# jkulhanek/viewformer

Hardware: NVIDIA H100
Metric: novel views/sec (128x128, 9-ctx) (higher is better)
Workload: dtype f32 encoder (bit-exact codes) + bf16 transformer/decoder

## Files before the change

### viewformer_b200/csrc/vf_tc_gemm.cu

```cuda
#include "vf_wgmma.cuh"
#include <stdlib.h>

namespace {
using namespace vftc;

constexpr int BLOCK_M = 128;
constexpr int ROW_BYTES = 128;
constexpr int A_STAGE_BYTES = BLOCK_M * ROW_BYTES;
constexpr int NUM_EPI_WARPS = 8;
constexpr int NUM_MMA_THREADS = 32 * NUM_EPI_WARPS;
constexpr int NUM_THREADS = NUM_MMA_THREADS + 128;

struct TcParams {
    CUtensorMap tmA, tmB;
    int conv;
    int M, Ncols;
    int num_k_blocks;
    int batch2;
    int tiles_m, tiles_n, total_tiles;
    int a_bm1, a_bm2, b_bm1, b_bm2;
    int TW, TH, TN, tiles_x, tiles_y, OH, OW, Nimg, cin_blocks, bk_elems;
    int tap_dy[9], tap_dx[9], tap_coff[9];
    int gemm_koff;
    int causal_block, causal_skip_n;
    float alpha;
    const float* bias;
    int bias_mode, act;
    const float* residual;
    float* C_f32;
    __nv_bfloat16* C_bf16;
    long long ldc, c_sb1, c_sb2;
    int vec_ok;
    int halo;
    double* gn_sums;
    int gn_groups, gn_cpg, gn_rows_per_img;
    int exact;
    int exact_kc;
    int exact_clog;
    int exact_kpp;
    int exact_lo_b;
    const float2* norm_mr;
    const float* norm_gamma;
    const float* norm_beta;
    int norm_groups, norm_cpg, norm_swish;
};

constexpr float EXACT_LO_SCALE = 1.0f / 2048.0f;

struct TileInfo {
    int m0, n0, b1, b2, img0, oy0, ox0, nkb;
    bool skip;
};

__device__ __forceinline__ TileInfo decode_tile(const TcParams& p, int t, int block_n) {
    TileInfo ti;
    const int n_tile = t % p.tiles_n;
    const int r = t / p.tiles_n;
    const int m_tile = r % p.tiles_m;
    const int bz = r / p.tiles_m;
    ti.b1 = bz / p.batch2;
    ti.b2 = bz % p.batch2;
    ti.m0 = m_tile * BLOCK_M;
    ti.n0 = n_tile * block_n;
    ti.nkb = p.num_k_blocks;
    ti.skip = false;
    if (p.causal_block > 0) {
        const int lim = ((ti.m0 + BLOCK_M - 1) / p.causal_block + 1) * p.causal_block;
        if (p.causal_skip_n) {
            ti.skip = ti.n0 >= lim;
        } else {
            const int kb = (lim + p.bk_elems - 1) / p.bk_elems;
            if (kb < ti.nkb) ti.nkb = kb;
        }
    }
    ti.img0 = ti.oy0 = ti.ox0 = 0;
    if (p.conv) {
        const int tx = m_tile % p.tiles_x;
        const int q = m_tile / p.tiles_x;
        ti.img0 = (q / p.tiles_y) * p.TN;
        ti.oy0 = (q % p.tiles_y) * p.TH;
        ti.ox0 = tx * p.TW;
    }
    return ti;
}

constexpr int HALO_BYTES = 23552;
__host__ __device__ constexpr int halo_buffers(bool exact) { return exact ? 4 : 2; }
__host__ __device__ constexpr int halo_slots(bool exact) { return exact ? 4 : 6; }
__host__ __device__ constexpr int operand_bytes(int stages, int stage_bytes, int b_stage_bytes, bool exact) {
    return stages * stage_bytes > halo_buffers(exact) * HALO_BYTES + halo_slots(exact) * b_stage_bytes
               ? stages * stage_bytes
               : halo_buffers(exact) * HALO_BYTES + halo_slots(exact) * b_stage_bytes;
}
constexpr int MAX_STAGES = 8;
template <int kBlockN, int kStages, bool kExact>
__host__ __device__ constexpr int tc_smem_bytes() {
    return operand_bytes(kStages, A_STAGE_BYTES + kBlockN * ROW_BYTES, kBlockN * ROW_BYTES, kExact) +
           NUM_EPI_WARPS * 32 * (kBlockN / 2 + 4) * 4  + 1024  + 8 * (2 * MAX_STAGES + 8) ;
}

__device__ __forceinline__ void prefetch_residual_l2(const TcParams& p, const TileInfo& ti, int block_n) {
    const int tw = min(p.TW, p.OW - ti.ox0);
    const uint32_t bytes = (uint32_t)(((long long)(tw - 1) * p.ldc + block_n) * 4);
    for (int r = 0; r < p.TN * p.TH; ++r) {
        const int img = ti.img0 + r / p.TH, oy = ti.oy0 + r % p.TH;
        if (img >= p.Nimg || oy >= p.OH) continue;
        const float* src = p.residual + ((long long)(img * p.OH + oy) * p.OW + ti.ox0) * p.ldc + ti.n0;
        asm volatile("cp.async.bulk.prefetch.L2.global [%0], %1;" ::"l"(src), "r"(bytes) : "memory");
    }
}

__device__ __forceinline__ void normalise_halo(const TcParams& p, uint8_t* tile, int cb, int img, int oy0, int ox0, int tid) {
    const int rows = (p.TW + 2) * (p.TH + 2);
    for (int idx = tid; idx < rows * 8; idx += NUM_MMA_THREADS) {
        const int r = idx >> 3, pc = idx & 7;
        const int py = r / (p.TW + 2), px = r - py * (p.TW + 2);
        const int iy = oy0 - 1 + py, ix = ox0 - 1 + px;
        if (iy < 0 || iy >= p.OH || ix < 0 || ix >= p.OW) continue;
        const int c0 = cb * 64 + ((pc ^ (r & 7)) << 3);
        uint4* ptr = reinterpret_cast<uint4*>(tile + r * ROW_BYTES + pc * 16);
        const uint4 v = *ptr;
        uint32_t w[4] = {v.x, v.y, v.z, v.w};
#pragma unroll
        for (int k = 0; k < 4; ++k) {
            const int c = c0 + 2 * k;
            const float2 ma = __ldg(p.norm_mr + (img * p.norm_groups + c / p.norm_cpg));
            const float2 mb = __ldg(p.norm_mr + (img * p.norm_groups + (c + 1) / p.norm_cpg));
            const float sa = ma.y * __ldg(p.norm_gamma + c), sb = mb.y * __ldg(p.norm_gamma + c + 1);
            float a = __uint_as_float(w[k] << 16), b = __uint_as_float(w[k] & 0xffff0000u);
            a = fmaf(a, sa, __ldg(p.norm_beta + c) - ma.x * sa);
            b = fmaf(b, sb, __ldg(p.norm_beta + c + 1) - mb.x * sb);
            if (p.norm_swish == 1) {
                a = __fdividef(a, 1.0f + __expf(-a));
                b = __fdividef(b, 1.0f + __expf(-b));
            }
            __nv_bfloat162 o = __floats2bfloat162_rn(a, b);
            w[k] = *reinterpret_cast<uint32_t*>(&o);
            if (p.norm_swish == 2) {
                uint32_t h, th;
                asm("mul.rn.bf16x2 %0, %1, %2;" : "=r"(h) : "r"(w[k]), "r"(0x3f003f00u));
                asm("tanh.approx.bf16x2 %0, %1;" : "=r"(th) : "r"(h));
                asm("fma.rn.bf16x2 %0, %1, %2, %1;" : "=r"(w[k]) : "r"(h), "r"(th));
            }
        }
        *ptr = make_uint4(w[0], w[1], w[2], w[3]);
    }
}

template <int kBlockN, int kStages, WgKind kKind>
__global__ void __launch_bounds__(NUM_THREADS, 1) tc_gemm_kernel(const __grid_constant__ TcParams p) {
    constexpr int B_STAGE_BYTES = kBlockN * ROW_BYTES;
    constexpr int STAGE_BYTES = A_STAGE_BYTES + B_STAGE_BYTES;
    constexpr int K_STEPS = 4;
    constexpr int HALF_N = kBlockN / 2;
    constexpr int STG_LD = HALF_N + 4;
    constexpr int STG_BYTES = NUM_EPI_WARPS * 32 * STG_LD * 4;
    constexpr int NACC = kBlockN / 2;
    constexpr bool kExact = kKind == F16;

    extern __shared__ uint8_t smem_raw[];
    uint8_t* smem = reinterpret_cast<uint8_t*>((reinterpret_cast<uintptr_t>(smem_raw) + 1023) & ~(uintptr_t)1023);
    constexpr int OPER_BYTES = operand_bytes(kStages, STAGE_BYTES, B_STAGE_BYTES, kExact);
    float* staging = reinterpret_cast<float*>(smem + OPER_BYTES);
    uint64_t* full_bar = reinterpret_cast<uint64_t*>(smem + OPER_BYTES + STG_BYTES);
    uint64_t* empty_bar = full_bar + MAX_STAGES;
    constexpr int NHB = halo_buffers(kExact);
    uint64_t* a_full_bar = empty_bar + MAX_STAGES;
    uint64_t* a_empty_bar = a_full_bar + NHB;
    constexpr int NG = kStages;
    constexpr int NGH = halo_slots(kExact);
    uint8_t* halo_b_base = smem + NHB * HALO_BYTES;

    const int warp = threadIdx.x >> 5;
    const int lane = threadIdx.x & 31;

    if (threadIdx.x == 0) {
        prefetch_tmap(&p.tmA);
        prefetch_tmap(&p.tmB);
        for (int s = 0; s < MAX_STAGES; ++s) {
            mbar_init(&full_bar[s], 1);
            mbar_init(&empty_bar[s], NUM_MMA_THREADS);
        }
        for (int a = 0; a < NHB; ++a) {
            mbar_init(&a_full_bar[a], 1);
            mbar_init(&a_empty_bar[a], NUM_MMA_THREADS);
        }
        mbar_fence_init();
    }
    __syncthreads();

    if (warp >= NUM_EPI_WARPS) {
        setmaxnreg_dec<40>();
        if (warp == NUM_EPI_WARPS && elect_one()) {
            int stage = 0;
            uint32_t phase = 0;
            int ab = 0;
            uint32_t aphase = 0, tpar = 0;
            for (int t = blockIdx.x; t < p.total_tiles; t += gridDim.x, tpar ^= 1) {
                const TileInfo ti = decode_tile(p, t, kBlockN);
                if (ti.skip) continue;
                const uint32_t halo_bytes = (uint32_t)((p.TW + 2) * (p.TH + 2)) * ROW_BYTES;
                if (kExact && p.halo) {
                    auto load_halves = [&](int h) {
                        for (int cb = 0; cb < p.cin_blocks; ++cb) {
                            const int hb = 2 * h + cb;
                            mbar_wait(&a_empty_bar[hb], tpar ^ 1, "vf_tc_gemm producer(halo)");
                            mbar_expect_tx(&a_full_bar[hb], halo_bytes);
                            tma_load_4d(smem + hb * HALO_BYTES, &p.tmA, &a_full_bar[hb], (h ? 0 : p.exact_clog) + cb * p.bk_elems,
                                        ti.ox0 - 1, ti.oy0 - 1, ti.img0);
                        }
                    };
                    load_halves(0);
                    if (p.residual && p.vec_ok && ti.n0 + kBlockN <= p.Ncols) prefetch_residual_l2(p, ti, kBlockN);
                    int j = 0, tap = 0, cb = 0;
                    for (int kb = 0; kb < ti.nkb; ++kb) {
                        if (kb == NGH) load_halves(1);
                        mbar_wait(&empty_bar[stage], phase ^ 1, "vf_tc_gemm producer");
                        mbar_expect_tx(&full_bar[stage], (uint32_t)B_STAGE_BYTES);
                        tma_load_4d(halo_b_base + stage * B_STAGE_BYTES, &p.tmB, &full_bar[stage],
                                    ((tap * 2 + (j == 1 ? 1 : 0)) * p.cin_blocks + cb) * p.bk_elems, ti.n0, 0, 0);
                        if (++cb == p.cin_blocks) { cb = 0; if (++tap == 9) { tap = 0; ++j; } }
                        if (++stage == NGH) { stage = 0; phase ^= 1; }
                    }
                    continue;
                }
                if (p.halo) {
                    const int nkb = 9 * p.cin_blocks;
                    int tap = 0, cb = 0;
                    for (int kb = 0; kb < nkb; ++kb) {
                        mbar_wait(&empty_bar[stage], phase ^ 1, "vf_tc_gemm producer");
                        mbar_expect_tx(&full_bar[stage], (uint32_t)B_STAGE_BYTES);
                        if (tap == 0) {
                            mbar_wait(&a_empty_bar[ab], aphase ^ 1, "vf_tc_gemm producer(halo)");
                            mbar_expect_tx(&a_full_bar[ab], halo_bytes);
                            tma_load_4d(smem + ab * HALO_BYTES, &p.tmA, &a_full_bar[ab], cb * p.bk_elems, ti.ox0 - 1, ti.oy0 - 1, ti.img0);
                            if (++ab == 2) { ab = 0; aphase ^= 1; }
                        }
                        tma_load_4d(halo_b_base + stage * B_STAGE_BYTES, &p.tmB, &full_bar[stage], (tap * p.cin_blocks + cb) * p.bk_elems,
                                    ti.n0, 0, 0);
                        if (++tap == 9) { tap = 0; ++cb; }
                        if (++stage == NGH) { stage = 0; phase ^= 1; }
                    }
                    continue;
                }
                if (kExact && p.conv && p.residual && p.vec_ok && ti.n0 + kBlockN <= p.Ncols) prefetch_residual_l2(p, ti, kBlockN);
                for (int kb = 0; kb < ti.nkb; ++kb) {
                    mbar_wait(&empty_bar[stage], phase ^ 1, "vf_tc_gemm producer");
                    mbar_expect_tx(&full_bar[stage], (uint32_t)STAGE_BYTES);
                    uint8_t* sa = smem + stage * STAGE_BYTES;
                    uint8_t* sb = sa + A_STAGE_BYTES;
                    int kcoord_b = kb * p.bk_elems;
                    if (p.conv) {
                        int kbr = kb, a_half = 0;
                        if (p.exact) {
                            const int j = kb / p.exact_kpp;
                            kbr = kb - j * p.exact_kpp;
                            a_half = (j == 0) ? p.exact_clog : 0;
                            const int tap_ = kbr / p.cin_blocks, cb_ = kbr - tap_ * p.cin_blocks;
                            kcoord_b = ((tap_ * 2 + (j == 1 ? 1 : 0)) * p.cin_blocks + cb_) * p.bk_elems;
                        }
                        const int tap = kbr / p.cin_blocks;
                        const int cb = kbr - tap * p.cin_blocks;
                        tma_load_4d(sa, &p.tmA, &full_bar[stage], a_half + p.tap_coff[tap] + cb * p.bk_elems, ti.ox0 + p.tap_dx[tap],
                                    ti.oy0 + p.tap_dy[tap], ti.img0);
                    } else {
                        int kcoord_a = kb * p.bk_elems;
                        if (p.exact) {
                            const int j = kb / p.exact_kpp, kbr = kb - j * p.exact_kpp;
                            kcoord_a = (j == 0 ? p.exact_clog : 0) + kbr * p.bk_elems;
                            kcoord_b = (j == 1 ? p.exact_lo_b : 0) + kbr * p.bk_elems;
                        }
                        if (p.gemm_koff) kcoord_a += p.tap_coff[ti.b1];
                        tma_load_4d(sa, &p.tmA, &full_bar[stage], kcoord_a, ti.m0, ti.b2 * p.a_bm2, ti.b1 * p.a_bm1);
                    }
                    tma_load_4d(sb, &p.tmB, &full_bar[stage], kcoord_b, ti.n0, ti.b2 * p.b_bm2, ti.b1 * p.b_bm1);
                    if (++stage == NG) { stage = 0; phase ^= 1; }
                }
            }
        }
        return;
    }

    setmaxnreg_inc<232>();
    const int wg = warp >> 2;
    const int quarter = warp & 3;
    const int col_half = warp >> 2;
    float* stg = staging + warp * (32 * STG_LD);
    int stage = 0, ab = 0;
    uint32_t phase = 0, aphase = 0, tpar = 0;

    const bool col_split = kExact && p.halo && p.TW == 16;
    auto to_staging = [&](const float (&v)[NACC], float sc) {
        const int r_lo = 64 * wg + 16 * (warp & 3) + (lane >> 2);
#pragma unroll
        for (int j = 0; j < NACC / 4; ++j) {
#pragma unroll
            for (int h = 0; h < 2; ++h) {
                const int r = col_split ? 16 * (2 * (warp & 3) + h) + 8 * wg + (lane >> 2) : r_lo + 8 * h;
                const int c = 8 * j + 2 * (lane & 3);
                float* dst = staging + ((c / HALF_N) * 4 + (r >> 5)) * (32 * STG_LD) + (r & 31) * STG_LD + (c % HALF_N);
                *reinterpret_cast<float2*>(dst) = make_float2(v[4 * j + 2 * h] * sc, v[4 * j + 2 * h + 1] * sc);
            }
        }
    };

    for (int t = blockIdx.x; t < p.total_tiles; t += gridDim.x, tpar ^= 1) {
        const TileInfo ti = decode_tile(p, t, kBlockN);
        if (ti.skip) continue;

        float acc[NACC];
        float csum[kExact ? NACC : 1];
        auto k_loop = [&]() {
            const int nkb = (p.halo && !kExact) ? 9 * p.cin_blocks : ti.nkb;
            const int nsmall = p.exact ? 2 * p.exact_kpp / p.exact_kc : 0;
            int prev_stage = -1, prev_halo = -1, in_chunk = 0, ck = 0, tap = 0, j = 0, cb = 0;
            bool fresh = true;
            uint32_t a_base = 0;
            const uint32_t pitch = (uint32_t)(p.TW + 2);
            const uint32_t wg_rows = p.TW == 16 ? 8u : 8u * pitch;
            auto retire_prev = [&]() {
                if (prev_stage >= 0) mbar_arrive(&empty_bar[prev_stage]);
                if (prev_halo >= 0) mbar_arrive(&a_empty_bar[prev_halo]);
                prev_stage = prev_halo = -1;
            };
#pragma unroll 1
            for (int kb = 0; kb < nkb; ++kb) {
                uint64_t adesc, bdesc;
                int this_halo = (p.halo && tap == 8) ? ab : -1;
                if (kExact && p.halo) {
                    const int hb = (j == 0 ? 0 : 2) + cb;
                    if (tap == 0 && j < 2) mbar_wait(&a_full_bar[hb], tpar, "vf_tc_gemm mma(halo)");
                    this_halo = (tap == 8 && j != 1) ? hb : -1;
                    mbar_wait(&full_bar[stage], phase, "vf_tc_gemm mma");
                    const uint32_t a_addr = smem_u32(smem + hb * HALO_BYTES) +
                                            ((uint32_t)(tap / 3) * pitch + (uint32_t)(tap % 3) + (uint32_t)wg * wg_rows) * ROW_BYTES;
                    adesc = sw128_desc(a_addr, pitch * ROW_BYTES);
                    bdesc = sw128_desc(smem_u32(halo_b_base + stage * B_STAGE_BYTES));
                } else if (p.halo) {
                    if (tap == 0) {
                        mbar_wait(&a_full_bar[ab], aphase, "vf_tc_gemm mma(halo)");
                        a_base = smem_u32(smem + ab * HALO_BYTES);
                        if (!kExact && p.norm_mr) {
                            normalise_halo(p, smem + ab * HALO_BYTES, kb / 9, ti.img0, ti.oy0, ti.ox0, threadIdx.x);
                            fence_async_smem();
                            named_sync(1, NUM_MMA_THREADS);
                        }
                    }
                    mbar_wait(&full_bar[stage], phase, "vf_tc_gemm mma");
                    const uint32_t a_addr = a_base + ((uint32_t)(tap / 3) * pitch + (uint32_t)(tap % 3) + (uint32_t)(8 * wg) * pitch) * ROW_BYTES;
                    adesc = sw128_desc(a_addr, pitch * ROW_BYTES);
                    bdesc = sw128_desc(smem_u32(halo_b_base + stage * B_STAGE_BYTES));
                } else {
                    mbar_wait(&full_bar[stage], phase, "vf_tc_gemm mma");
                    const uint32_t sa = smem_u32(smem + stage * STAGE_BYTES);
                    adesc = sw128_desc(sa + (uint32_t)(wg * 64 * ROW_BYTES));
                    bdesc = sw128_desc(sa + A_STAGE_BYTES);
                }
                wgmma_fence();
#pragma unroll
                for (int k = 0; k < K_STEPS; ++k)
                    wgmma_ss<kBlockN, kKind>(acc, adesc + (uint64_t)(2 * k), bdesc + (uint64_t)(2 * k), (fresh && k == 0) ? 0u : 1u);
                wgmma_commit();
                fresh = false;
                wgmma_wait<1>();
                retire_prev();
                prev_stage = stage;
                prev_halo = this_halo;
                if (kExact && p.halo) {
                    if (++stage == NGH) { stage = 0; phase ^= 1; }
                    if (++cb == p.cin_blocks) { cb = 0; if (++tap == 9) { tap = 0; ++j; } }
                } else if (p.halo) {
                    if (++stage == NGH) { stage = 0; phase ^= 1; }
                    if (++tap == 9) { tap = 0; if (++ab == 2) { ab = 0; aphase ^= 1; } }
                } else {
                    if (++stage == NG) { stage = 0; phase ^= 1; }
                }
                if (kExact && ++in_chunk == p.exact_kc) {
                    in_chunk = 0;
                    wgmma_wait<0>();
                    reg_fence(acc);
                    const float sc = (ck < nsmall ? EXACT_LO_SCALE : 1.0f) * p.alpha;
                    if (ck == 0) {
#pragma unroll
                        for (int i = 0; i < NACC; ++i) csum[i] = acc[i] * sc;
                    } else {
#pragma unroll
                        for (int i = 0; i < NACC; ++i) csum[i] = fmaf(acc[i], sc, csum[i]);
                    }
                    ++ck;
                    fresh = true;
                }
            }
            wgmma_wait<0>();
            reg_fence(acc);
            retire_prev();
        };
        if constexpr (kExact) k_loop();

        const int row = quarter * 32 + lane;
        long long my_off;
        int my_ok, gm;
        if (p.conv) {
            const int lx = row % p.TW;
            const int q = row / p.TW;
            const int ly = q % p.TH;
            const int ln = q / p.TH;
            const int img = ti.img0 + ln, oy = ti.oy0 + ly, ox = ti.ox0 + lx;
            my_ok = (img < p.Nimg) && (oy < p.OH) && (ox < p.OW);
            gm = (img * p.OH + oy) * p.OW + ox;
            my_off = (long long)gm * p.ldc;
        } else {
            gm = ti.m0 + row;
            my_ok = gm < p.M;
            my_off = (long long)ti.b1 * p.c_sb1 + (long long)ti.b2 * p.c_sb2 + (long long)gm * p.ldc;
        }
        const float bias_m = (p.bias_mode == VF_BIAS_M && my_ok) ? __ldg(p.bias + gm) : 0.f;

        constexpr int VPR = HALF_N / 4;
        constexpr int RPI = 32 / VPR;
        constexpr int ITERS = 32 / RPI;
        const int r_sub = lane / VPR;
        const int c_ln = (lane % VPR) * 4;
        const int n_ln = ti.n0 + col_half * HALF_N + c_ln;
        const bool fast = p.vec_ok && (ti.n0 + kBlockN <= p.Ncols);
        auto residual_at = [&](int i) {
            const int rr = i * RPI + r_sub;
            const int ok = __shfl_sync(0xffffffffu, my_ok, rr);
            const long long off_row = __shfl_sync(0xffffffffu, my_off, rr);
            const long long o = ok ? off_row + n_ln : (long long)n_ln;
            return __ldg(reinterpret_cast<const float4*>(p.residual + o));
        };
        constexpr int RB = kExact ? ITERS / 2 : ITERS;
        float4 resv[RB];
        auto load_residual = [&](int i0) {
            if (fast && p.residual) {
#pragma unroll
                for (int i = 0; i < RB; ++i) resv[i] = residual_at(i0 + i);
            }
        };
        if constexpr (!kExact) load_residual(0);
        float4 bias4 = make_float4(0.f, 0.f, 0.f, 0.f);
        if (fast && p.bias_mode == VF_BIAS_N) bias4 = __ldg(reinterpret_cast<const float4*>(p.bias + n_ln));

        if constexpr (!kExact) k_loop();
        named_sync(1, NUM_MMA_THREADS);
        if constexpr (kExact) to_staging(csum, 1.0f);
        else to_staging(acc, p.alpha);
        named_sync(1, NUM_MMA_THREADS);

        if (fast) {
            float gs = 0.f, gq = 0.f;
#pragma unroll
            for (int i = 0; i < ITERS; ++i) {
                if (kExact && i % RB == 0) load_residual(i);
                const int rr = i * RPI + r_sub;
                const int ok = __shfl_sync(0xffffffffu, my_ok, rr);
                const long long off_row = __shfl_sync(0xffffffffu, my_off, rr);
                const float bm = __shfl_sync(0xffffffffu, bias_m, rr);
                float4 v = *reinterpret_cast<const float4*>(stg + rr * STG_LD + c_ln);
                if (p.bias_mode == VF_BIAS_N) { v.x += bias4.x; v.y += bias4.y; v.z += bias4.z; v.w += bias4.w; }
                else { v.x += bm; v.y += bm; v.z += bm; v.w += bm; }
                if (p.act == VF_ACT_GELU_ERF) { v.x = vf_gelu_erf(v.x); v.y = vf_gelu_erf(v.y); v.z = vf_gelu_erf(v.z); v.w = vf_gelu_erf(v.w); }
                if (p.residual) {
                    const float4 r = resv[i % RB];
                    v.x += r.x; v.y += r.y; v.z += r.z; v.w += r.w;
                }
                if (ok) {
                    gs += (v.x + v.y) + (v.z + v.w);
                    gq += (v.x * v.x + v.y * v.y) + (v.z * v.z + v.w * v.w);
                    const long long off = off_row + n_ln;
                    if (p.C_f32) *reinterpret_cast<float4*>(p.C_f32 + off) = v;
                    if (p.C_bf16) {
                        __nv_bfloat162 lo = __floats2bfloat162_rn(v.x, v.y), hi = __floats2bfloat162_rn(v.z, v.w);
                        uint2 u;
                        u.x = *reinterpret_cast<uint32_t*>(&lo);
                        u.y = *reinterpret_cast<uint32_t*>(&hi);
                        *reinterpret_cast<uint2*>(p.C_bf16 + off) = u;
                    }
                }
            }
            if (p.gn_sums) {
                const unsigned okmask = __ballot_sync(0xffffffffu, my_ok);
#pragma unroll
                for (int o = VPR; o < 32; o <<= 1) {
                    gs += __shfl_xor_sync(0xffffffffu, gs, o);
                    gq += __shfl_xor_sync(0xffffffffu, gq, o);
                }
                const int lpg = p.gn_cpg >> 2;
                for (int o = 1; o < lpg; o <<= 1) {
                    gs += __shfl_xor_sync(0xffffffffu, gs, o);
                    gq += __shfl_xor_sync(0xffffffffu, gq, o);
                }
                const int gm_first = __shfl_sync(0xffffffffu, gm, okmask ? (__ffs(okmask) - 1) : 0);
                if (okmask && r_sub == 0 && (lane % lpg) == 0) {
                    const long long slot = ((long long)(gm_first / p.gn_rows_per_img) * p.gn_groups + n_ln / p.gn_cpg) * 2;
                    atomicAdd(p.gn_sums + slot, (double)gs);
                    atomicAdd(p.gn_sums + slot + 1, (double)gq);
                }
            }
        } else {
#pragma unroll 1
            for (int rr = 0; rr < 32; ++rr) {
                const int ok = __shfl_sync(0xffffffffu, my_ok, rr);
                const long long off_row = __shfl_sync(0xffffffffu, my_off, rr);
                const float bm = __shfl_sync(0xffffffffu, bias_m, rr);
                if (!ok) continue;
                for (int c = lane; c < HALF_N; c += 32) {
                    const int n = ti.n0 + col_half * HALF_N + c;
                    if (n >= p.Ncols) continue;
                    float x = stg[rr * STG_LD + c];
                    x += (p.bias_mode == VF_BIAS_N) ? __ldg(p.bias + n) : bm;
                    if (p.act == VF_ACT_GELU_ERF) x = vf_gelu_erf(x);
                    const long long off = off_row + n;
                    if (p.residual) x += __ldg(p.residual + off);
                    if (p.C_f32) p.C_f32[off] = x;
                    if (p.C_bf16) p.C_bf16[off] = __float2bfloat16(x);
                }
            }
        }
    }
}

int make_tmap(CUtensorMap* tm, int dtype, const void* base, const uint64_t dims[4], const uint64_t strides_bytes[3],
              const uint32_t box[4]) {
    EncodeTiledFn fn = encode_fn();
    if (!fn) { vf_set_error("vf_tc_gemm: cuTensorMapEncodeTiled unavailable"); return VF_ERR_CUDA; }
    cuuint64_t gdim[4] = {dims[0], dims[1], dims[2], dims[3]};
    cuuint64_t gstr[3] = {strides_bytes[0], strides_bytes[1], strides_bytes[2]};
    cuuint32_t bx[4] = {box[0], box[1], box[2], box[3]};
    cuuint32_t es[4] = {1, 1, 1, 1};
    CUresult r = fn(tm, dtype == VF_BF16 ? CU_TENSOR_MAP_DATA_TYPE_BFLOAT16 : CU_TENSOR_MAP_DATA_TYPE_FLOAT32, 4,
                    const_cast<void*>(base), gdim, gstr, bx, es, CU_TENSOR_MAP_INTERLEAVE_NONE, CU_TENSOR_MAP_SWIZZLE_128B,
                    CU_TENSOR_MAP_L2_PROMOTION_L2_256B, CU_TENSOR_MAP_FLOAT_OOB_FILL_NONE);
    if (r != CUDA_SUCCESS) {
        vf_set_error("vf_tc_gemm: cuTensorMapEncodeTiled failed (%d): dims=[%llu,%llu,%llu,%llu] strides=[%llu,%llu,%llu] box=[%u,%u,%u,%u]",
                     (int)r, (unsigned long long)dims[0], (unsigned long long)dims[1], (unsigned long long)dims[2],
                     (unsigned long long)dims[3], (unsigned long long)strides_bytes[0], (unsigned long long)strides_bytes[1],
                     (unsigned long long)strides_bytes[2], box[0], box[1], box[2], box[3]);
        return VF_ERR_CUDA;
    }
    return VF_OK;
}

template <int kBlockN, int kStages, WgKind kKind>
int launch(const TcParams& prm, dim3 grid, cudaStream_t st) {
    constexpr int smem = tc_smem_bytes<kBlockN, kStages, kKind == F16>();
    static_assert(kStages <= MAX_STAGES, "ring depth");
    static_assert(smem <= 232448, "shared memory budget");
    static vf_per_device_flag configured_pd;
    bool& configured = configured_pd.current();
    if (!configured) {
        cudaError_t e = cudaFuncSetAttribute(tc_gemm_kernel<kBlockN, kStages, kKind>, cudaFuncAttributeMaxDynamicSharedMemorySize, smem);
        if (e != cudaSuccess) { vf_set_error("vf_tc_gemm: cudaFuncSetAttribute: %s", cudaGetErrorString(e)); return VF_ERR_CUDA; }
        configured = true;
    }
    tc_gemm_kernel<kBlockN, kStages, kKind><<<grid, NUM_THREADS, smem, st>>>(prm);
    VF_CHECK_LAUNCH("vf_tc_gemm");
    return VF_OK;
}

template <int kBlockN, int kStages>
int launch_kind(const TcParams& prm, WgKind kind, dim3 grid, cudaStream_t st) {
    if (kind == TF32) return launch<kBlockN, kStages, TF32>(prm, grid, st);
    if (kind == F16) return launch<kBlockN, kStages, F16>(prm, grid, st);
    return launch<kBlockN, kStages, BF16>(prm, grid, st);
}

}

extern "C" int vf_tc_gemm(const vf_tc_gemm_t* q, vf_stream_t s) {
    VF_CHECK_ARG(q && q->A && q->B, "vf_tc_gemm: null operand");
    VF_CHECK_ARG(q->C_f32 || q->C_bf16, "vf_tc_gemm: no output");
    VF_CHECK_ARG(q->ab_dtype == VF_BF16 || q->ab_dtype == VF_F32 || q->ab_dtype == VF_F16X2, "vf_tc_gemm: bad dtype");
    const bool exact = q->ab_dtype == VF_F16X2;
    if (exact) {
        VF_CHECK_ARG(q->C_f32 && !q->C_bf16 && !q->norm_mean_rstd && q->causal_block == 0,
                     "vf_tc_gemm: VF_F16X2 (exact split-fp16) operands need an fp32 output and no causal / fused-norm options");
        if (q->conv) VF_CHECK_ARG(q->Ctot % 2 == 0 && q->alpha == 1.0f, "vf_tc_gemm: exact conv needs [hi | lo] channels and alpha = 1");
        else VF_CHECK_ARG(q->K % 64 == 0 && q->exact_lo_a >= q->K && q->exact_lo_b >= q->K && q->exact_lo_a % 8 == 0 && q->exact_lo_b % 8 == 0,
                          "vf_tc_gemm: exact GEMM needs K %% 64 == 0 and lo-half offsets >= K (K=%d lo_a=%lld lo_b=%lld)", q->K,
                          (long long)q->exact_lo_a, (long long)q->exact_lo_b);
    }
    VF_CHECK_ARG(q->bias_mode == VF_BIAS_NONE || q->bias, "vf_tc_gemm: bias pointer missing");
    VF_CHECK_ARG(!q->norm_mean_rstd || q->conv, "vf_tc_gemm: fused input GroupNorm is a convolution option");
    const bool tf32 = q->ab_dtype == VF_F32;
    const int tm_dtype = tf32 ? VF_F32 : VF_BF16;
    const int es = tf32 ? 4 : 2;
    const int bk = ROW_BYTES / es;

    TcParams prm;
    memset(&prm, 0, sizeof(prm));
    prm.conv = q->conv;
    prm.Ncols = q->Ncols;
    prm.bk_elems = bk;
    prm.alpha = q->alpha;
    prm.bias = q->bias;
    prm.bias_mode = q->bias_mode;
    prm.act = q->act;
    prm.residual = q->residual;
    prm.C_f32 = q->C_f32;
    prm.C_bf16 = reinterpret_cast<__nv_bfloat16*>(q->C_bf16);
    prm.ldc = q->ldc;
    prm.causal_block = q->causal_block;
    prm.causal_skip_n = q->causal_skip_n;

    const int block_n = (q->Ncols > 64) ? 128 : 64;
    const int b_box_rows = block_n;
    dim3 grid;
    int rc;
    if (q->conv) {
        VF_CHECK_ARG(q->ntaps >= 1 && q->ntaps <= 9, "vf_tc_gemm: ntaps");
        VF_CHECK_ARG(q->Cin % bk == 0 && q->Ctot % (16 / es) == 0, "vf_tc_gemm: conv Cin=%d must be a multiple of %d", q->Cin, bk);
        VF_CHECK_ARG(q->causal_block == 0, "vf_tc_gemm: causal with conv");
        int TW = q->OW >= 16 ? 16 : (q->OW >= 8 ? 8 : (q->OW >= 4 ? 4 : (q->OW >= 2 ? 2 : 1)));
        int TH = 128 / TW;
        if (TH > q->OH) { TH = 1; while (TH * 2 <= q->OH) TH *= 2; }
        int TN = 128 / (TW * TH);
        bool halo = q->ntaps == 9 && q->OH == q->H && q->OW == q->W &&
                    (exact ? q->Ctot == 2 * q->Cin && q->Cin <= 2 * bk && TN == 1 && TW >= 8
                           : q->Ctot == q->Cin && q->OH >= 16 && q->OW >= 8);
        for (int t = 0; halo && t < 9; ++t) halo = q->tap_dy[t] == t / 3 - 1 && q->tap_dx[t] == t % 3 - 1 && q->tap_coff[t] == 0;
        if (halo && !exact) { TW = 8; TH = 16; TN = 1; }
        prm.halo = halo ? 1 : 0;
        if (q->norm_mean_rstd) {
            VF_CHECK_ARG(halo && q->ab_dtype == VF_BF16 && q->H >= 32 && q->Ncols % 128 == 0 && q->Cin % 64 == 0,
                         "vf_tc_gemm: fused input GroupNorm needs a 3x3 stride-1 bf16 conv on a map >= 32 rows (Cin %% 64 == 0, Cout %% 128 == 0)");
            VF_CHECK_ARG(q->norm_gamma && q->norm_beta && q->norm_groups > 0 && q->Cin % q->norm_groups == 0,
                         "vf_tc_gemm: fused input GroupNorm needs gamma, beta and a group count dividing Cin");
            prm.norm_mr = reinterpret_cast<const float2*>(q->norm_mean_rstd);
            prm.norm_gamma = q->norm_gamma;
            prm.norm_beta = q->norm_beta;
            prm.norm_groups = q->norm_groups;
            prm.norm_cpg = q->Cin / q->norm_groups;
            prm.norm_swish = q->norm_swish;
        }
        VF_CHECK_ARG(TW * TH * TN == 128 && TN <= 256, "vf_tc_gemm: cannot tile %dx%d output", q->OH, q->OW);
        prm.TW = TW; prm.TH = TH; prm.TN = TN;
        prm.tiles_x = (q->OW + TW - 1) / TW;
        prm.tiles_y = (q->OH + TH - 1) / TH;
        prm.OH = q->OH; prm.OW = q->OW; prm.Nimg = q->N;
        prm.cin_blocks = q->Cin / bk;
        prm.num_k_blocks = q->ntaps * prm.cin_blocks;
        if (exact) {
            prm.exact = 1;
            prm.exact_kpp = prm.num_k_blocks;
            prm.exact_clog = q->Ctot / 2;
            prm.exact_kc = (prm.num_k_blocks % 3 == 0) ? 3 : 1;
// ... 99 lines not shown
```

Measured before the change: 247.9.

## Add warp-specialized epilogue warpgroup for exact F16 halo conv GEMM

```diff
diff --git a/viewformer_b200/csrc/vf_tc_gemm.cu b/viewformer_b200/csrc/vf_tc_gemm.cu
--- a/viewformer_b200/csrc/vf_tc_gemm.cu
+++ b/viewformer_b200/csrc/vf_tc_gemm.cu
@@ -7,9 +7,14 @@
 constexpr int BLOCK_M = 128;
 constexpr int ROW_BYTES = 128;
 constexpr int A_STAGE_BYTES = BLOCK_M * ROW_BYTES;
-constexpr int NUM_EPI_WARPS = 8;
-constexpr int NUM_MMA_THREADS = 32 * NUM_EPI_WARPS;
-constexpr int NUM_THREADS = NUM_MMA_THREADS + 128;
+constexpr int NUM_MMA_WARPS = 8;
+constexpr int NUM_MMA_THREADS = 32 * NUM_MMA_WARPS;
+constexpr int NUM_EPI_THREADS = 128;
+constexpr int STG_SLICES = 8;
+__host__ __device__ constexpr int num_threads(bool split) { return NUM_MMA_THREADS + (split ? NUM_EPI_THREADS : 0) + 128; }
+constexpr int MMA_REGS = 176, EPI_REGS = 120, PRODUCER_REGS = 40, MMA_EPI_REGS = 232;
+static_assert(NUM_MMA_THREADS * MMA_REGS + NUM_EPI_THREADS * EPI_REGS + 128 * PRODUCER_REGS <= 512 * 128, "register budget");
+static_assert(NUM_MMA_THREADS * MMA_EPI_REGS + 128 * PRODUCER_REGS <= 384 * 168, "register budget");
 
 struct TcParams {
     CUtensorMap tmA, tmB;
@@ -96,7 +101,7 @@
 template <int kBlockN, int kStages, bool kExact>
 __host__ __device__ constexpr int tc_smem_bytes() {
     return operand_bytes(kStages, A_STAGE_BYTES + kBlockN * ROW_BYTES, kBlockN * ROW_BYTES, kExact) +
-           NUM_EPI_WARPS * 32 * (kBlockN / 2 + 4) * 4  + 1024  + 8 * (2 * MAX_STAGES + 8) ;
+           STG_SLICES * 32 * (kBlockN / 2 + 4) * 4  + 1024  + 8 * (2 * MAX_STAGES + 10) ;
 }
 
 __device__ __forceinline__ void prefetch_residual_l2(const TcParams& p, const TileInfo& ti, int block_n) {
@@ -147,14 +152,14 @@
     }
 }
 
-template <int kBlockN, int kStages, WgKind kKind>
-__global__ void __launch_bounds__(NUM_THREADS, 1) tc_gemm_kernel(const __grid_constant__ TcParams p) {
+template <int kBlockN, int kStages, WgKind kKind, bool kSplitEpilogue>
+__global__ void __launch_bounds__(num_threads(kSplitEpilogue), 1) tc_gemm_kernel(const __grid_constant__ TcParams p) {
     constexpr int B_STAGE_BYTES = kBlockN * ROW_BYTES;
     constexpr int STAGE_BYTES = A_STAGE_BYTES + B_STAGE_BYTES;
     constexpr int K_STEPS = 4;
     constexpr int HALF_N = kBlockN / 2;
     constexpr int STG_LD = HALF_N + 4;
-    constexpr int STG_BYTES = NUM_EPI_WARPS * 32 * STG_LD * 4;
+    constexpr int STG_BYTES = STG_SLICES * 32 * STG_LD * 4;
     constexpr int NACC = kBlockN / 2;
     constexpr bool kExact = kKind == F16;
 
@@ -167,6 +172,8 @@
     constexpr int NHB = halo_buffers(kExact);
     uint64_t* a_full_bar = empty_bar + MAX_STAGES;
     uint64_t* a_empty_bar = a_full_bar + NHB;
+    uint64_t* stg_full_bar = a_empty_bar + NHB;
+    uint64_t* stg_empty_bar = stg_full_bar + 1;
     constexpr int NG = kStages;
     constexpr int NGH = halo_slots(kExact);
     uint8_t* halo_b_base = smem + NHB * HALO_BYTES;
@@ -185,13 +192,16 @@
             mbar_init(&a_full_bar[a], 1);
             mbar_init(&a_empty_bar[a], NUM_MMA_THREADS);
         }
+        mbar_init(stg_full_bar, NUM_MMA_THREADS);
+        mbar_init(stg_empty_bar, NUM_EPI_THREADS);
         mbar_fence_init();
     }
     __syncthreads();
 
-    if (warp >= NUM_EPI_WARPS) {
-        setmaxnreg_dec<40>();
-        if (warp == NUM_EPI_WARPS && elect_one()) {
+    constexpr int EPI_WARP0 = NUM_MMA_WARPS, PRODUCER_WARP0 = kSplitEpilogue ? NUM_MMA_WARPS + NUM_EPI_THREADS / 32 : NUM_MMA_WARPS;
+    if (warp >= PRODUCER_WARP0) {
+        setmaxnreg_dec<PRODUCER_REGS>();
+        if (warp == PRODUCER_WARP0 && elect_one()) {
             int stage = 0;
             uint32_t phase = 0;
             int ab = 0;
@@ -281,13 +291,9 @@
         return;
     }
 
-    setmaxnreg_inc<232>();
     const int wg = warp >> 2;
-    const int quarter = warp & 3;
-    const int col_half = warp >> 2;
-    float* stg = staging + warp * (32 * STG_LD);
     int stage = 0, ab = 0;
-    uint32_t phase = 0, aphase = 0, tpar = 0;
+    uint32_t phase = 0, aphase = 0, tpar = 0, sphase = 0;
 
     const bool col_split = kExact && p.halo && p.TW == 16;
     auto to_staging = [&](const float (&v)[NACC], float sc) {
@@ -304,99 +310,103 @@
         }
     };
 
-    for (int t = blockIdx.x; t < p.total_tiles; t += gridDim.x, tpar ^= 1) {
-        const TileInfo ti = decode_tile(p, t, kBlockN);
-        if (ti.skip) continue;
-
+    auto mma_tile = [&](const TileInfo& ti, auto&& before_staging) {
         float acc[NACC];
         float csum[kExact ? NACC : 1];
-        auto k_loop = [&]() {
-            const int nkb = (p.halo && !kExact) ? 9 * p.cin_blocks : ti.nkb;
-            const int nsmall = p.exact ? 2 * p.exact_kpp / p.exact_kc : 0;
-            int prev_stage = -1, prev_halo = -1, in_chunk = 0, ck = 0, tap = 0, j = 0, cb = 0;
-            bool fresh = true;
-            uint32_t a_base = 0;
-            const uint32_t pitch = (uint32_t)(p.TW + 2);
-            const uint32_t wg_rows = p.TW == 16 ? 8u : 8u * pitch;
-            auto retire_prev = [&]() {
-                if (prev_stage >= 0) mbar_arrive(&empty_bar[prev_stage]);
-                if (prev_halo >= 0) mbar_arrive(&a_empty_bar[prev_halo]);
-                prev_stage = prev_halo = -1;
-            };
+        const int nkb = (p.halo && !kExact) ? 9 * p.cin_blocks : ti.nkb;
+        const int nsmall = p.exact ? 2 * p.exact_kpp / p.exact_kc : 0;
+        int prev_stage = -1, prev_halo = -1, in_chunk = 0, ck = 0, tap = 0, j = 0, cb = 0;
+        bool fresh = true;
+        uint32_t a_base = 0;
+        const uint32_t pitch = (uint32_t)(p.TW + 2);
+        const uint32_t wg_rows = p.TW == 16 ? 8u : 8u * pitch;
+        auto retire_prev = [&]() {
+            if (prev_stage >= 0) mbar_arrive(&empty_bar[prev_stage]);
+            if (prev_halo >= 0) mbar_arrive(&a_empty_bar[prev_halo]);
+            prev_stage = prev_halo = -1;
+        };
 #pragma unroll 1
-            for (int kb = 0; kb < nkb; ++kb) {
-                uint64_t adesc, bdesc;
-                int this_halo = (p.halo && tap == 8) ? ab : -1;
-                if (kExact && p.halo) {
-                    const int hb = (j == 0 ? 0 : 2) + cb;
-                    if (tap == 0 && j < 2) mbar_wait(&a_full_bar[hb], tpar, "vf_tc_gemm mma(halo)");
-                    this_halo = (tap == 8 && j != 1) ? hb : -1;
-                    mbar_wait(&full_bar[stage], phase, "vf_tc_gemm mma");
-                    const uint32_t a_addr = smem_u32(smem + hb * HALO_BYTES) +
-                                            ((uint32_t)(tap / 3) * pitch + (uint32_t)(tap % 3) + (uint32_t)wg * wg_rows) * ROW_BYTES;
-                    adesc = sw128_desc(a_addr, pitch * ROW_BYTES);
-                    bdesc = sw128_desc(smem_u32(halo_b_base + stage * B_STAGE_BYTES));
-                } else if (p.halo) {
-                    if (tap == 0) {
-                        mbar_wait(&a_full_bar[ab], aphase, "vf_tc_gemm mma(halo)");
-                        a_base = smem_u32(smem + ab * HALO_BYTES);
-                        if (!kExact && p.norm_mr) {
-                            normalise_halo(p, smem + ab * HALO_BYTES, kb / 9, ti.img0, ti.oy0, ti.ox0, threadIdx.x);
-                            fence_async_smem();
-                            named_sync(1, NUM_MMA_THREADS);
-                        }
-                    }
-                    mbar_wait(&full_bar[stage], phase, "vf_tc_gemm mma");
-                    const uint32_t a_addr = a_base + ((uint32_t)(tap / 3) * pitch + (uint32_t)(tap % 3) + (uint32_t)(8 * wg) * pitch) * ROW_BYTES;
-                    adesc = sw128_desc(a_addr, pitch * ROW_BYTES);
-                    bdesc = sw128_desc(smem_u32(halo_b_base + stage * B_STAGE_BYTES));
+        for (int kb = 0; kb < nkb; ++kb) {
+            uint64_t adesc, bdesc;
+            int this_halo = (p.halo && tap == 8) ? ab : -1;
+            if (kExact && p.halo) {
+                const int hb = (j == 0 ? 0 : 2) + cb;
+                if (tap == 0 && j < 2) mbar_wait(&a_full_bar[hb], tpar, "vf_tc_gemm mma(halo)");
+                this_halo = (tap == 8 && j != 1) ? hb : -1;
+                mbar_wait(&full_bar[stage], phase, "vf_tc_gemm mma");
+                const uint32_t a_addr = smem_u32(smem + hb * HALO_BYTES) +
+                                        ((uint32_t)(tap / 3) * pitch + (uint32_t)(tap % 3) + (uint32_t)wg * wg_rows) * ROW_BYTES;
+                adesc = sw128_desc(a_addr, pitch * ROW_BYTES);
+                bdesc = sw128_desc(smem_u32(halo_b_base + stage * B_STAGE_BYTES));
+            } else if (p.halo) {
+                if (tap == 0) {
+                    mbar_wait(&a_full_bar[ab], aphase, "vf_tc_gemm mma(halo)");
+                    a_base = smem_u32(smem + ab * HALO_BYTES);
+                    if (!kExact && p.norm_mr) {
+                        normalise_halo(p, smem + ab * HALO_BYTES, kb / 9, ti.img0, ti.oy0, ti.ox0, threadIdx.x);
+                        fence_async_smem();
+                        named_sync(1, NUM_MMA_THREADS);
+                    }
+                }
+                mbar_wait(&full_bar[stage], phase, "vf_tc_gemm mma");
+                const uint32_t a_addr = a_base + ((uint32_t)(tap / 3) * pitch + (uint32_t)(tap % 3) + (uint32_t)(8 * wg) * pitch) * ROW_BYTES;
+                adesc = sw128_desc(a_addr, pitch * ROW_BYTES);
+                bdesc = sw128_desc(smem_u32(halo_b_base + stage * B_STAGE_BYTES));
+            } else {
+                mbar_wait(&full_bar[stage], phase, "vf_tc_gemm mma");
+                const uint32_t sa = smem_u32(smem + stage * STAGE_BYTES);
+                adesc = sw128_desc(sa + (uint32_t)(wg * 64 * ROW_BYTES));
+                bdesc = sw128_desc(sa + A_STAGE_BYTES);
+            }
+            wgmma_fence();
+#pragma unroll
+            for (int k = 0; k < K_STEPS; ++k)
+                wgmma_ss<kBlockN, kKind>(acc, adesc + (uint64_t)(2 * k), bdesc + (uint64_t)(2 * k), (fresh && k == 0) ? 0u : 1u);
+            wgmma_commit();
+            fresh = false;
+            wgmma_wait<1>();
+            retire_prev();
+            prev_stage = stage;
+            prev_halo = this_halo;
+            if (kExact && p.halo) {
+                if (++stage == NGH) { stage = 0; phase ^= 1; }
+                if (++cb == p.cin_blocks) { cb = 0; if (++tap == 9) { tap = 0; ++j; } }
+            } else if (p.halo) {
+                if (++stage == NGH) { stage = 0; phase ^= 1; }
+                if (++tap == 9) { tap = 0; if (++ab == 2) { ab = 0; aphase ^= 1; } }
+            } else {
+                if (++stage == NG) { stage = 0; phase ^= 1; }
+            }
+            if (kExact && ++in_chunk == p.exact_kc) {
+                in_chunk = 0;
+                wgmma_wait<0>();
+                reg_fence(acc);
+                const float sc = (ck < nsmall ? EXACT_LO_SCALE : 1.0f) * p.alpha;
+                if (ck == 0) {
+#pragma unroll
+                    for (int i = 0; i < NACC; ++i) csum[i] = acc[i] * sc;
                 } else {
-                    mbar_wait(&full_bar[stage], phase, "vf_tc_gemm mma");
-                    const uint32_t sa = smem_u32(smem + stage * STAGE_BYTES);
-                    adesc = sw128_desc(sa + (uint32_t)(wg * 64 * ROW_BYTES));
-                    bdesc = sw128_desc(sa + A_STAGE_BYTES);
+#pragma unroll
+                    for (int i = 0; i < NACC; ++i) csum[i] = fmaf(acc[i], sc, csum[i]);
                 }
-                wgmma_fence();
-#pragma unroll
-                for (int k = 0; k < K_STEPS; ++k)
-                    wgmma_ss<kBlockN, kKind>(acc, adesc + (uint64_t)(2 * k), bdesc + (uint64_t)(2 * k), (fresh && k == 0) ? 0u : 1u);
-                wgmma_commit();
-                fresh = false;
-                wgmma_wait<1>();
-                retire_prev();
-                prev_stage = stage;
-                prev_halo = this_halo;
-                if (kExact && p.halo) {
-                    if (++stage == NGH) { stage = 0; phase ^= 1; }
-                    if (++cb == p.cin_blocks) { cb = 0; if (++tap == 9) { tap = 0; ++j; } }
-                } else if (p.halo) {
-                    if (++stage == NGH) { stage = 0; phase ^= 1; }
-                    if (++tap == 9) { tap = 0; if (++ab == 2) { ab = 0; aphase ^= 1; } }
-                } else {
-                    if (++stage == NG) { stage = 0; phase ^= 1; }
-                }
-                if (kExact && ++in_chunk == p.exact_kc) {
-                    in_chunk = 0;
-                    wgmma_wait<0>();
-                    reg_fence(acc);
-                    const float sc = (ck < nsmall ? EXACT_LO_SCALE : 1.0f) * p.alpha;
-                    if (ck == 0) {
-#pragma unroll
-                        for (int i = 0; i < NACC; ++i) csum[i] = acc[i] * sc;
-                    } else {
-#pragma unroll
-                        for (int i = 0; i < NACC; ++i) csum[i] = fmaf(acc[i], sc, csum[i]);
-                    }
-                    ++ck;
-                    fresh = true;
-                }
-            }
-            wgmma_wait<0>();
-            reg_fence(acc);
-            retire_prev();
-        };
-        if constexpr (kExact) k_loop();
-
+                ++ck;
+                fresh = true;
+            }
+        }
+        wgmma_wait<0>();
+        reg_fence(acc);
+        retire_prev();
+        before_staging();
+        if constexpr (kExact) to_staging(csum, 1.0f);
+        else to_staging(acc, p.alpha);
+    };
+
+    auto epilogue_tile = [&](const TileInfo& ti, int quarter, int h0, int nh, auto&& wait_staging) {
+    constexpr int VPR = HALF_N / 4;
+    constexpr int RPI = 32 / VPR;
+    constexpr int ITERS = 32 / RPI;
+    const int r_sub = lane / VPR;
+    const int c_ln = (lane % VPR) * 4;
         const int row = quarter * 32 + lane;
         long long my_off;
         int my_ok, gm;
@@ -416,106 +426,141 @@
         }
         const float bias_m = (p.bias_mode == VF_BIAS_M && my_ok) ? __ldg(p.bias + gm) : 0.f;
 
-        constexpr int VPR = HALF_N / 4;
-        constexpr int RPI = 32 / VPR;
-        constexpr int ITERS = 32 / RPI;
-        const int r_sub = lane / VPR;
-        const int c_ln = (lane % VPR) * 4;
-        const int n_ln = ti.n0 + col_half * HALF_N + c_ln;
         const bool fast = p.vec_ok && (ti.n0 + kBlockN <= p.Ncols);
-        auto residual_at = [&](int i) {
+        auto residual_at = [&](int col_half, int i) {
             const int rr = i * RPI + r_sub;
             const int ok = __shfl_sync(0xffffffffu, my_ok, rr);
             const long long off_row = __shfl_sync(0xffffffffu, my_off, rr);
+            const int n_ln = ti.n0 + col_half * HALF_N + c_ln;
             const long long o = ok ? off_row + n_ln : (long long)n_ln;
             return __ldg(reinterpret_cast<const float4*>(p.residual + o));
         };
-        constexpr int RB = kExact ? ITERS / 2 : ITERS;
+        constexpr bool kLoadAfterWait = kExact && !kSplitEpilogue;
+        constexpr int RB = kLoadAfterWait ? ITERS / 2 : ITERS;
         float4 resv[RB];
         auto load_residual = [&](int i0) {
             if (fast && p.residual) {
 #pragma unroll
-                for (int i = 0; i < RB; ++i) resv[i] = residual_at(i0 + i);
+                for (int i = 0; i < RB; ++i) resv[i] = residual_at(h0, i0 + i);
             }
         };
-        if constexpr (!kExact) load_residual(0);
-        float4 bias4 = make_float4(0.f, 0.f, 0.f, 0.f);
-        if (fast && p.bias_mode == VF_BIAS_N) bias4 = __ldg(reinterpret_cast<const float4*>(p.bias + n_ln));
-
-        if constexpr (!kExact) k_loop();
-        named_sync(1, NUM_MMA_THREADS);
-        if constexpr (kExact) to_staging(csum, 1.0f);
-        else to_staging(acc, p.alpha);
-        named_sync(1, NUM_MMA_THREADS);
-
-        if (fast) {
-            float gs = 0.f, gq = 0.f;
-#pragma unroll
-            for (int i = 0; i < ITERS; ++i) {
-                if (kExact && i % RB == 0) load_residual(i);
-                const int rr = i * RPI + r_sub;
-                const int ok = __shfl_sync(0xffffffffu, my_ok, rr);
-                const long long off_row = __shfl_sync(0xffffffffu, my_off, rr);
-                const float bm = __shfl_sync(0xffffffffu, bias_m, rr);
-                float4 v = *reinterpret_cast<const float4*>(stg + rr * STG_LD + c_ln);
-                if (p.bias_mode == VF_BIAS_N) { v.x += bias4.x; v.y += bias4.y; v.z += bias4.z; v.w += bias4.w; }
-                else { v.x += bm; v.y += bm; v.z += bm; v.w += bm; }
-                if (p.act == VF_ACT_GELU_ERF) { v.x = vf_gelu_erf(v.x); v.y = vf_gelu_erf(v.y); v.z = vf_gelu_erf(v.z); v.w = vf_gelu_erf(v.w); }
-                if (p.residual) {
-                    const float4 r = resv[i % RB];
-                    v.x += r.x; v.y += r.y; v.z += r.z; v.w += r.w;
+        if constexpr (!kLoadAfterWait) load_residual(0);
+        wait_staging();
+
+#pragma unroll
+        for (int col_half = h0; col_half < h0 + nh; ++col_half) {
+            const float* stg = staging + (col_half * 4 + quarter) * (32 * STG_LD);
+            const int n_ln = ti.n0 + col_half * HALF_N + c_ln;
+            if (fast) {
+                float4 bias4 = make_float4(0.f, 0.f, 0.f, 0.f);
+                if (p.bias_mode == VF_BIAS_N) bias4 = __ldg(reinterpret_cast<const float4*>(p.bias + n_ln));
+                float gs = 0.f, gq = 0.f;
+#pragma unroll
+                for (int i = 0; i < ITERS; ++i) {
+                    if (kLoadAfterWait && i % RB == 0) load_residual(i);
+                    const int rr = i * RPI + r_sub;
+                    const int ok = __shfl_sync(0xffffffffu, my_ok, rr);
+                    const long long off_row = __shfl_sync(0xffffffffu, my_off, rr);
+                    const float bm = __shfl_sync(0xffffffffu, bias_m, rr);
+                    float4 v = *reinterpret_cast<const float4*>(stg + rr * STG_LD + c_ln);
+                    if (p.bias_mode == VF_BIAS_N) { v.x += bias4.x; v.y += bias4.y; v.z += bias4.z; v.w += bias4.w; }
+                    else { v.x += bm; v.y += bm; v.z += bm; v.w += bm; }
+                    if (p.act == VF_ACT_GELU_ERF) { v.x = vf_gelu_erf(v.x); v.y = vf_gelu_erf(v.y); v.z = vf_gelu_erf(v.z); v.w = vf_gelu_erf(v.w); }
+                    if (p.residual) {
+                        const float4 r = resv[i % RB];
+                        if (!kLoadAfterWait && col_half + 1 < h0 + nh) resv[i] = residual_at(col_half + 1, i);
+                        v.x += r.x; v.y += r.y; v.z += r.z; v.w += r.w;
+                    }
+                    if (ok) {
+                        gs += (v.x + v.y) + (v.z + v.w);
+                        gq += __fmaf_rn(v.y, v.y, __fmul_rn(v.x, v.x)) + __fmaf_rn(v.w, v.w, __fmul_rn(v.z, v.z));
+                        const long long off = off_row + n_ln;
+                        if (p.C_f32) *reinterpret_cast<float4*>(p.C_f32 + off) = v;
+                        if (p.C_bf16) {
+                            __nv_bfloat162 lo = __floats2bfloat162_rn(v.x, v.y), hi = __floats2bfloat162_rn(v.z, v.w);
+                            uint2 u;
+                            u.x = *reinterpret_cast<uint32_t*>(&lo);
+                            u.y = *reinterpret_cast<uint32_t*>(&hi);
+                            *reinterpret_cast<uint2*>(p.C_bf16 + off) = u;
+                        }
+                    }
                 }
-                if (ok) {
-                    gs += (v.x + v.y) + (v.z + v.w);
-                    gq += (v.x * v.x + v.y * v.y) + (v.z * v.z + v.w * v.w);
-                    const long long off = off_row + n_ln;
-                    if (p.C_f32) *reinterpret_cast<float4*>(p.C_f32 + off) = v;
-                    if (p.C_bf16) {
-                        __nv_bfloat162 lo = __floats2bfloat162_rn(v.x, v.y), hi = __floats2bfloat162_rn(v.z, v.w);
-                        uint2 u;
-                        u.x = *reinterpret_cast<uint32_t*>(&lo);
-                        u.y = *reinterpret_cast<uint32_t*>(&hi);
-                        *reinterpret_cast<uint2*>(p.C_bf16 + off) = u;
+                if (p.gn_sums) {
+                    const unsigned okmask = __ballot_sync(0xffffffffu, my_ok);
+#pragma unroll
+                    for (int o = VPR; o < 32; o <<= 1) {
+                        gs += __shfl_xor_sync(0xffffffffu, gs, o);
+                        gq += __shfl_xor_sync(0xffffffffu, gq, o);
+                    }
+                    const int lpg = p.gn_cpg >> 2;
+                    for (int o = 1; o < lpg; o <<= 1) {
+                        gs += __shfl_xor_sync(0xffffffffu, gs, o);
+                        gq += __shfl_xor_sync(0xffffffffu, gq, o);
+                    }
+                    const int gm_first = __shfl_sync(0xffffffffu, gm, okmask ? (__ffs(okmask) - 1) : 0);
+                    if (okmask && r_sub == 0 && (lane % lpg) == 0) {
+                        const long long slot = ((long long)(gm_first / p.gn_rows_per_img) * p.gn_groups + n_ln / p.gn_cpg) * 2;
+                        atomicAdd(p.gn_sums + slot, (double)gs);
+                        atomicAdd(p.gn_sums + slot + 1, (double)gq);
                     }
                 }
-            }
-            if (p.gn_sums) {
-                const unsigned okmask = __ballot_sync(0xffffffffu, my_ok);
-#pragma unroll
-                for (int o = VPR; o < 32; o <<= 1) {
-                    gs += __shfl_xor_sync(0xffffffffu, gs, o);
-                    gq += __shfl_xor_sync(0xffffffffu, gq, o);
+            } else {
+#pragma unroll 1
+                for (int rr = 0; rr < 32; ++rr) {
+                    const int ok = __shfl_sync(0xffffffffu, my_ok, rr);
+                    const long long off_row = __shfl_sync(0xffffffffu, my_off, rr);
+                    const float bm = __shfl_sync(0xffffffffu, bias_m, rr);
+                    if (!ok) continue;
+                    for (int c = lane; c < HALF_N; c += 32) {
+                        const int n = ti.n0 + col_half * HALF_N + c;
+                        if (n >= p.Ncols) continue;
+                        float x = stg[rr * STG_LD + c];
+                        x += (p.bias_mode == VF_BIAS_N) ? __ldg(p.bias + n) : bm;
+                        if (p.act == VF_ACT_GELU_ERF) x = vf_gelu_erf(x);
+                        const long long off = off_row + n;
+                        if (p.residual) x += __ldg(p.residual + off);
+                        if (p.C_f32) p.C_f32[off] = x;
+                        if (p.C_bf16) p.C_bf16[off] = __float2bfloat16(x);
+                    }
                 }
-                const int lpg = p.gn_cpg >> 2;
-                for (int o = 1; o < lpg; o <<= 1) {
-                    gs += __shfl_xor_sync(0xffffffffu, gs, o);
-                    gq += __shfl_xor_sync(0xffffffffu, gq, o);
-                }
-                const int gm_first = __shfl_sync(0xffffffffu, gm, okmask ? (__ffs(okmask) - 1) : 0);
-                if (okmask && r_sub == 0 && (lane % lpg) == 0) {
-                    const long long slot = ((long long)(gm_first / p.gn_rows_per_img) * p.gn_groups + n_ln / p.gn_cpg) * 2;
-                    atomicAdd(p.gn_sums + slot, (double)gs);
-                    atomicAdd(p.gn_sums + slot + 1, (double)gq);
-                }
-            }
-        } else {
-#pragma unroll 1
-            for (int rr = 0; rr < 32; ++rr) {
-                const int ok = __shfl_sync(0xffffffffu, my_ok, rr);
-                const long long off_row = __shfl_sync(0xffffffffu, my_off, rr);
-                const float bm = __shfl_sync(0xffffffffu, bias_m, rr);
-                if (!ok) continue;
-                for (int c = lane; c < HALF_N; c += 32) {
-                    const int n = ti.n0 + col_half * HALF_N + c;
-                    if (n >= p.Ncols) continue;
-                    float x = stg[rr * STG_LD + c];
-                    x += (p.bias_mode == VF_BIAS_N) ? __ldg(p.bias + n) : bm;
-                    if (p.act == VF_ACT_GELU_ERF) x = vf_gelu_erf(x);
-                    const long long off = off_row + n;
-                    if (p.residual) x += __ldg(p.residual + off);
-                    if (p.C_f32) p.C_f32[off] = x;
-                    if (p.C_bf16) p.C_bf16[off] = __float2bfloat16(x);
-                }
+            }
+        }
+    };
+
+    if constexpr (kSplitEpilogue) {
+        if (warp >= EPI_WARP0) {
+            setmaxnreg_dec<EPI_REGS>();
+            for (int t = blockIdx.x; t < p.total_tiles; t += gridDim.x) {
+                const TileInfo ti = decode_tile(p, t, kBlockN);
+                if (ti.skip) continue;
+                epilogue_tile(ti, warp - EPI_WARP0, 0, 2, [&]() { mbar_wait(stg_full_bar, sphase, "vf_tc_gemm epilogue"); });
+                mbar_arrive(stg_empty_bar);
+                sphase ^= 1;
+            }
+            return;
+        }
+        setmaxnreg_inc<MMA_REGS>();
+        for (int t = blockIdx.x; t < p.total_tiles; t += gridDim.x, tpar ^= 1) {
+            const TileInfo ti = decode_tile(p, t, kBlockN);
+            if (ti.skip) continue;
+            mma_tile(ti, [&]() { mbar_wait(stg_empty_bar, sphase ^ 1, "vf_tc_gemm mma(staging)"); });
+            mbar_arrive(stg_full_bar);
+            sphase ^= 1;
+        }
+    } else {
+        setmaxnreg_inc<MMA_EPI_REGS>();
+        for (int t = blockIdx.x; t < p.total_tiles; t += gridDim.x, tpar ^= 1) {
+            const TileInfo ti = decode_tile(p, t, kBlockN);
+            if (ti.skip) continue;
+            auto k_loop_to_staging = [&]() {
+                mma_tile(ti, [&]() { named_sync(1, NUM_MMA_THREADS); });
+                named_sync(1, NUM_MMA_THREADS);
+            };
+            if constexpr (kExact) {
+                k_loop_to_staging();
+                epilogue_tile(ti, warp & 3, warp >> 2, 1, []() {});
+            } else {
+                epilogue_tile(ti, warp & 3, warp >> 2, 1, k_loop_to_staging);
             }
         }
     }
@@ -542,7 +587,7 @@
     return VF_OK;
 }
 
-template <int kBlockN, int kStages, WgKind kKind>
+template <int kBlockN, int kStages, WgKind kKind, bool kSplit = false>
 int launch(const TcParams& prm, dim3 grid, cudaStream_t st) {
     constexpr int smem = tc_smem_bytes<kBlockN, kStages, kKind == F16>();
     static_assert(kStages <= MAX_STAGES, "ring depth");
@@ -550,11 +595,11 @@
     static vf_per_device_flag configured_pd;
     bool& configured = configured_pd.current();
     if (!configured) {
-        cudaError_t e = cudaFuncSetAttribute(tc_gemm_kernel<kBlockN, kStages, kKind>, cudaFuncAttributeMaxDynamicSharedMemorySize, smem);
+        cudaError_t e = cudaFuncSetAttribute(tc_gemm_kernel<kBlockN, kStages, kKind, kSplit>, cudaFuncAttributeMaxDynamicSharedMemorySize, smem);
         if (e != cudaSuccess) { vf_set_error("vf_tc_gemm: cudaFuncSetAttribute: %s", cudaGetErrorString(e)); return VF_ERR_CUDA; }
         configured = true;
     }
-    tc_gemm_kernel<kBlockN, kStages, kKind><<<grid, NUM_THREADS, smem, st>>>(prm);
+    tc_gemm_kernel<kBlockN, kStages, kKind, kSplit><<<grid, num_threads(kSplit), smem, st>>>(prm);
     VF_CHECK_LAUNCH("vf_tc_gemm");
     return VF_OK;
 }
@@ -562,7 +607,12 @@
 template <int kBlockN, int kStages>
 int launch_kind(const TcParams& prm, WgKind kind, dim3 grid, cudaStream_t st) {
     if (kind == TF32) return launch<kBlockN, kStages, TF32>(prm, grid, st);
-    if (kind == F16) return launch<kBlockN, kStages, F16>(prm, grid, st);
+    if (kind == F16) {
+        if constexpr (kBlockN == 128) {
+            if (prm.halo && prm.OH <= 64) return launch<kBlockN, kStages, F16, true>(prm, grid, st);
+        }
+        return launch<kBlockN, kStages, F16>(prm, grid, st);
+    }
     return launch<kBlockN, kStages, BF16>(prm, grid, st);
 }
 
```

Result: no change. 246.8, median of 6 (-0.4%).
